# jjjkkyz/NU-NeRF

Measured on AMD Instinct MI355X. Metric: train rays/sec, higher is better.
Workload: dtype f32

## Files before the change

### nu_nerf_amd/csrc/gemm_epi.h

```cpp
#pragma once
#include "gemm.h"
#include <type_traits>

#define TBM 128
#define TBN 128
#define TBK 32
#define NT_LDS 36
#define NT_LDSH 40
#define NT_WPC 3

#define EPI_LDS 68

template <int EPI>
static __device__ inline float nu_epi_apply(float v, float bv, float h, float d, float ca, float& out2) {
    out2 = 0.f;
    if (EPI == NU_EPI_BIAS_NONE) return v + bv;
    if (EPI == NU_EPI_BIAS_RELU) return fmaxf(v + bv, 0.0f);
    if (EPI == NU_EPI_BIAS_SOFTPLUS) return nu_softplus100_fast(v + bv);
    if (EPI == NU_EPI_MUL_DRELU) return h > 0.0f ? v : 0.0f;
    if (EPI == NU_EPI_MUL_DSP) return v * (1.0f - nu_exp_m100(h));
    if (EPI == NU_EPI_Q_SP) {
        const float e = nu_exp_m100(h);
        out2 = v * d * 100.0f * e;
        return v * (1.0f - e);
    }
    if (EPI == NU_EPI_B_SP) return v * (1.0f - nu_exp_m100(h)) + ca;
    if (EPI == NU_EPI_B_RELU) return (h > 0.0f ? v : 0.0f) + ca;
    return v;
}

template <int EPI>
struct NtEpiArgs {
    float* C; float* C2; const float* bias; const float* H; const float* D; const float* Cadd;
    unsigned long long* mask;
    int zero_to, act_cols;
    bool vec_ok;
    bool c16, x16;
    static constexpr bool kMaskW = (EPI == NU_EPI_BIAS_RELU);
    static constexpr bool kMaskR = (EPI == NU_EPI_MUL_DRELU || EPI == NU_EPI_B_RELU);
    static constexpr bool kNeedH = (EPI == NU_EPI_MUL_DRELU || EPI == NU_EPI_MUL_DSP || EPI == NU_EPI_Q_SP ||
                                    EPI == NU_EPI_B_SP || EPI == NU_EPI_B_RELU);
    static constexpr bool kNeedD = (EPI == NU_EPI_Q_SP);
    static constexpr bool kNeedAdd = (EPI == NU_EPI_B_SP || EPI == NU_EPI_B_RELU);
    static constexpr bool kBias = (EPI <= NU_EPI_BIAS_SOFTPLUS);
};

template <int EPI, bool H16 = false>
static __device__ inline NtEpiArgs<EPI> nt_epi_args(const NuGemmNT& g, int z) {
    typedef NtEpiArgs<EPI> E;
    E a;
    a.c16 = H16 && (g.bf16 & NU_GEMM_C16) != 0;
    a.x16 = H16 && (g.bf16 & NU_GEMM_X16) != 0;
    const int ec = a.c16 ? 2 : 4, ex = a.x16 ? 2 : 4;
    auto off = [](const float* p, long long elems, int eb) { return reinterpret_cast<const float*>(reinterpret_cast<const char*>(p) + elems * eb); };
    a.C = const_cast<float*>(off(g.C, (long long)z * g.sC, ec));
    a.C2 = g.C2 ? const_cast<float*>(off(g.C2, (long long)z * g.sC2, ec)) : nullptr;
    a.bias = g.bias ? g.bias + (long long)z * g.sBias : nullptr;
    a.H = g.H ? off(g.H, (long long)z * g.sH, ex) : nullptr;
    a.D = g.D ? off(g.D, (long long)z * g.sD, ex) : nullptr;
    a.Cadd = g.Cadd ? off(g.Cadd, (long long)z * g.sCadd, ex) : nullptr;
    a.zero_to = g.zero_to > g.N ? g.zero_to : g.N;
    a.act_cols = g.act_cols > 0 ? g.act_cols : 0x7fffffff;
    a.mask = (E::kMaskW || E::kMaskR) ? g.mask : nullptr;
    const uintptr_t mc = a.c16 ? 7 : 15, mx = a.x16 ? 7 : 15;
    bool v = (((uintptr_t)a.C & mc) == 0) && ((g.ldc & 3) == 0);
    if (E::kNeedH) v = v && (((uintptr_t)a.H & mx) == 0) && ((g.ldh & 3) == 0);
    if (E::kNeedD) v = v && (((uintptr_t)a.D & mx) == 0) && ((g.ldd & 3) == 0) && (((uintptr_t)a.C2 & mc) == 0) && ((g.ldc2 & 3) == 0);
    if (E::kNeedAdd) v = v && (((uintptr_t)a.Cadd & mx) == 0) && ((g.ldadd & 3) == 0);
    a.vec_ok = v;
    return a;
}

static __device__ __forceinline__ f32x4 nu_bf16x4_to_f32(uint2 r) {
    f32x4 o;
    o[0] = __uint_as_float(r.x << 16); o[1] = __uint_as_float(r.x & 0xffff0000u);
    o[2] = __uint_as_float(r.y << 16); o[3] = __uint_as_float(r.y & 0xffff0000u);
    return o;
}
template <bool H16> static __device__ __forceinline__ f32x4 nt_ld4(const char* p, bool is16) {
    if (H16 && is16) return nu_bf16x4_to_f32(*reinterpret_cast<const uint2*>(p));
    return *reinterpret_cast<const f32x4*>(p);
}
template <bool H16> static __device__ __forceinline__ void nt_st4(char* p, f32x4 v, bool is16) {
// ... 6 lines not shown
}
template <bool H16> static __device__ __forceinline__ void nt_st1(float* base, long long idx, float v, bool is16) {
    if (H16 && is16) reinterpret_cast<__bf16*>(base)[idx] = (__bf16)v;
    else base[idx] = v;
}

template <int EPI>
static __device__ inline unsigned long long* nt_mask_words(const NtEpiArgs<EPI>& ea, const NuGemmNT& g, int mt, int nt, int z, int ntn, int wid) {
    const int ct = g.mask_ct0 + z * ntn + nt;
    return (ea.mask && ct < g.mask_nct) ? ea.mask + ((((long long)mt * g.mask_nct + ct) * 4 + wid) * 64) : nullptr;
}

template <int EPI, int NBH, bool H16 = false, int TMN = 2>
static __device__ __forceinline__ void nt_epilogue(const NuGemmNT& g, const NtEpiArgs<EPI>& ea, f32x16 (&acc)[TMN][2], float* scr,
                                                   int m0, int n0, unsigned long long* mwave, unsigned mlo, unsigned mhi,
                                                   int lane, int wid, int tm0 = 0) {
    typedef NtEpiArgs<EPI> E;
    constexpr bool kMaskW = E::kMaskW, kMaskR = E::kMaskR, kNeedH = E::kNeedH, kNeedD = E::kNeedD, kNeedAdd = E::kNeedAdd, kBias = E::kBias;
    float* const C = ea.C; float* const C2 = ea.C2;
    const float* const bias = ea.bias; const float* const H = ea.H; const float* const D = ea.D; const float* const Cadd = ea.Cadd;
    const int zero_to = ea.zero_to, act_cols = ea.act_cols;
    const bool vec_ok = ea.vec_ok;
    const bool c16 = H16 && ea.c16, x16 = H16 && ea.x16;
    const int ec = c16 ? 2 : 4, ex = x16 ? 2 : 4;
    const int li = lane & 31, lh = lane >> 5;
    const int wr = wid >> 1, wc = wid & 1;
    unsigned wlo = 0, whi = 0;
    const int colq = (lane & 15) * 4;
    const int gcol = n0 + wc * 64 + colq;
    float bv[4] = {0.f, 0.f, 0.f, 0.f};
    if (kBias && bias) {
#pragma unroll
        for (int e = 0; e < 4; ++e) bv[e] = (gcol + e < g.N) ? bias[gcol + e] : 0.f;
    }
    const bool full = vec_ok && (gcol + 3 < g.N) && (gcol + 3 < act_cols || gcol >= act_cols);
    const int wcol0 = n0 + wc * 64, wrow0 = m0 + wr * 64;
    const bool slab_full = vec_ok && (wrow0 + 64 <= g.M) && (wcol0 + 64 <= g.N) && (wcol0 + 64 <= act_cols || wcol0 >= act_cols);
    const bool slab_plain = kNeedH && wcol0 >= act_cols;
    const int uwid = __builtin_amdgcn_readfirstlane(wid);
    const long long urow0 = m0 + (uwid >> 1) * 64, ucol0 = n0 + (uwid & 1) * 64;
    const unsigned lrow = lane >> 4;
    char* const Cu = reinterpret_cast<char*>(C) + (urow0 * g.ldc + ucol0) * ec;
    char* const C2u = kNeedD ? reinterpret_cast<char*>(C2) + (urow0 * g.ldc2 + ucol0) * ec : nullptr;
    const char* const Hu = kNeedH ? reinterpret_cast<const char*>(H) + (urow0 * g.ldh + ucol0) * ex : nullptr;
    const char* const Du = kNeedD ? reinterpret_cast<const char*>(D) + (urow0 * g.ldd + ucol0) * ex : nullptr;
    const char* const Au = kNeedAdd ? reinterpret_cast<const char*>(Cadd) + (urow0 * g.ldadd + ucol0) * ex : nullptr;
    const unsigned oC = (lrow * (unsigned)g.ldc + (unsigned)colq) * (unsigned)ec, oC2 = (lrow * (unsigned)g.ldc2 + (unsigned)colq) * (unsigned)ec;
    const unsigned oH = (lrow * (unsigned)g.ldh + (unsigned)colq) * (unsigned)ex, oD = (lrow * (unsigned)g.ldd + (unsigned)colq) * (unsigned)ex;
    const unsigned oA = (lrow * (unsigned)g.ldadd + (unsigned)colq) * (unsigned)ex;
#pragma unroll
    for (int tt = 0; tt < TMN; ++tt) {
        const int tm = tm0 + tt;
#pragma unroll
        for (int tn = 0; tn < 2; ++tn)
#pragma unroll
            for (int r = 0; r < 16; ++r)
                scr[((r & 3) + 8 * (r >> 2) + 4 * lh) * EPI_LDS + tn * 32 + li] = acc[tt][tn][r];
        if (slab_full) {
            auto fast = [&](auto ub_c, auto pl_c, auto c16_c, auto x16_c) {
                constexpr bool UB = decltype(ub_c)::value, PL = decltype(pl_c)::value;
                constexpr bool c16 = decltype(c16_c)::value, x16 = decltype(x16_c)::value;
                constexpr int ec = c16 ? 2 : 4, ex = x16 ? 2 : 4;
                constexpr int NB = kNeedH ? NBH : 4;
#pragma unroll
                for (int hb = 0; hb < 8 / NB; ++hb) {
                    f32x4 v4[NB], h4[NB], d4[NB], c4v[NB];
#pragma unroll
                    for (int ii = 0; ii < NB; ++ii) {
                        const int i = hb * NB + ii;
                        const long long roff = (long long)(tm * 32 + i * 4);
                        v4[ii] = *reinterpret_cast<const f32x4*>(&scr[(i * 4 + (lane >> 4)) * EPI_LDS + colq]);
                        if (kNeedH && !PL && !UB) h4[ii] = nt_ld4<H16>(Hu + roff * g.ldh * ex + oH, x16);
                        if (kNeedD && !PL) d4[ii] = nt_ld4<H16>(Du + roff * g.ldd * ex + oD, x16);
                        if (kNeedAdd && !PL) c4v[ii] = nt_ld4<H16>(Au + roff * g.ldadd * ex + oA, x16);
                    }
#pragma unroll
                    for (int ii = 0; ii < NB; ++ii) {
                        const int i = hb * NB + ii;
                        const long long roff = (long long)(tm * 32 + i * 4);
                        f32x4 o4, o24;
#pragma unroll
                        for (int e = 0; e < 4; ++e) {
                            float o2 = 0.f;
                            const float v = g.alpha * v4[ii][e];
                            if constexpr (PL) {
                                o4[e] = v;
                            } else if constexpr (kMaskR && UB) {
                                const int src = (tm * 8 + i) * 4 + e;
                                const unsigned long long w = ((unsigned long long)(unsigned)__builtin_amdgcn_readlane(mhi, src) << 32) |
                                                             (unsigned)__builtin_amdgcn_readlane(mlo, src);
                                float sel;
                                asm("s_nop 1\n\tv_cndmask_b32_e64 %0, 0, %1, %2" : "=v"(sel) : "v"(v), "s"(w));
                                o4[e] = kNeedAdd ? sel + c4v[ii][e] : sel;
                            } else {
                                o4[e] = nu_epi_apply<EPI>(v, bv[e], kNeedH ? h4[ii][e] : 0.f, kNeedD ? d4[ii][e] : 0.f,
                                                          kNeedAdd ? c4v[ii][e] : 0.f, o2);
                            }
                            o24[e] = o2;
                        }
                        nt_st4<H16>(Cu + roff * g.ldc * ec + oC, o4, c16);
                        if (kNeedD) nt_st4<H16>(C2u + roff * g.ldc2 * ec + oC2, o24, c16);
                        if constexpr (kMaskW && UB) {
#pragma unroll
                            for (int e = 0; e < 4; ++e) {
                                const unsigned long long bits = __ballot(o4[e] > 0.f);
                                const bool mine = lane == (tm * 8 + i) * 4 + e;
                                wlo = mine ? (unsigned)bits : wlo;
                                whi = mine ? (unsigned)(bits >> 32) : whi;
                            }
                        }
                    }
                }
            };
            auto fast_w = [&](auto ub_c, auto pl_c) {
                constexpr bool kAux = kNeedH || kNeedD || kNeedAdd;
                if constexpr (H16) {
                    if (c16) {
                        if (kAux && x16) fast(ub_c, pl_c, std::true_type{}, std::true_type{});
                        else fast(ub_c, pl_c, std::true_type{}, std::false_type{});
                    } else {
                        if (kAux && x16) fast(ub_c, pl_c, std::false_type{}, std::true_type{});
                        else fast(ub_c, pl_c, std::false_type{}, std::false_type{});
                    }
                } else {
                    fast(ub_c, pl_c, std::false_type{}, std::false_type{});
                }
            };
            if (kNeedH && slab_plain) fast_w(std::false_type{}, std::true_type{});
            else if ((kMaskR || kMaskW) && mwave) fast_w(std::true_type{}, std::false_type{});
            else fast_w(std::false_type{}, std::false_type{});
        } else if (gcol < zero_to) {
#pragma unroll 4
            for (int i = 0; i < 8; ++i) {
                const int rl = i * 4 + (lane >> 4);
                const int row = m0 + wr * 64 + tm * 32 + rl;
                const f32x4 v4 = *reinterpret_cast<const f32x4*>(&scr[rl * EPI_LDS + colq]);
                bool pos[4] = {false, false, false, false};
                if (row < g.M) {
                if (full) {
                    f32x4 h4 = {0.f, 0.f, 0.f, 0.f}, d4 = h4, c4v = h4, o4, o24;
                    const bool plain = gcol >= act_cols;
                    if (kMaskR && mwave) {
                        if (!plain) {
#pragma unroll
                            for (int e = 0; e < 4; ++e) {
                                const int src = (tm * 8 + i) * 4 + e;
                                const unsigned lo = __builtin_amdgcn_readlane(mlo, src), hi = __builtin_amdgcn_readlane(mhi, src);
                                h4[e] = (((lane < 32 ? lo : hi) >> (lane & 31)) & 1u) ? 1.0f : 0.0f;
                            }
                        }
                    } else if (kNeedH && !plain) h4 = nt_ld4<H16>(reinterpret_cast<const char*>(H) + ((long long)row * g.ldh + gcol) * ex, x16);
                    if (kNeedD && !plain) d4 = nt_ld4<H16>(reinterpret_cast<const char*>(D) + ((long long)row * g.ldd + gcol) * ex, x16);
                    if (kNeedAdd && !plain) c4v = nt_ld4<H16>(reinterpret_cast<const char*>(Cadd) + ((long long)row * g.ldadd + gcol) * ex, x16);
#pragma unroll
                    for (int e = 0; e < 4; ++e) {
                        float o2;
                        const float v = g.alpha * v4[e];
                        o4[e] = (kNeedH && plain) ? v : nu_epi_apply<EPI>(v, bv[e], h4[e], d4[e], c4v[e], o2);
                        o24[e] = (kNeedH && plain) ? 0.f : o2;
                    }
                    nt_st4<H16>(reinterpret_cast<char*>(C) + ((long long)row * g.ldc + gcol) * ec, o4, c16);
                    if (kNeedD) nt_st4<H16>(reinterpret_cast<char*>(C2) + ((long long)row * g.ldc2 + gcol) * ec, o24, c16);
                    if (kMaskW) {
#pragma unroll
                        for (int e = 0; e < 4; ++e) pos[e] = o4[e] > 0.f;
                    }
                } else {
#pragma unroll
                    for (int e = 0; e < 4; ++e) {
                        const int col = gcol + e;
                        if (col >= zero_to) continue;
                        float out = 0.f, out2 = 0.f;
                        if (col < g.N) {
                            const float v = g.alpha * v4[e];
                            if (kNeedH && col >= act_cols) {
                                out = v;
                            } else {
                                const float h = kNeedH ? nt_ld1<H16>(H, (long long)row * g.ldh + col, x16) : 0.f;
                                const float d = kNeedD ? nt_ld1<H16>(D, (long long)row * g.ldd + col, x16) : 0.f;
                                const float ca = kNeedAdd ? nt_ld1<H16>(Cadd, (long long)row * g.ldadd + col, x16) : 0.f;
                                out = nu_epi_apply<EPI>(v, bv[e], h, d, ca, out2);
                            }
                        }
                        nt_st1<H16>(C, (long long)row * g.ldc + col, out, c16);
                        if (kNeedD) nt_st1<H16>(C2, (long long)row * g.ldc2 + col, out2, c16);
                    }
                }
                }
                if (kMaskW && mwave) {
#pragma unroll
                    for (int e = 0; e < 4; ++e) {
                        const unsigned long long bits = __ballot(pos[e]);
                        const bool mine = lane == (tm * 8 + i) * 4 + e;
                        wlo = mine ? (unsigned)bits : wlo;
                        whi = mine ? (unsigned)(bits >> 32) : whi;
                    }
                }
            }
        }
    }
    if (kMaskW && mwave && (TMN == 2 || (lane >> 5) == tm0)) mwave[lane] = ((unsigned long long)whi << 32) | wlo;
}

// ... 1 lines not shown
```

### nu_nerf_amd/csrc/gemm_nt.hip

```cpp
#include "gemm_epi.h"

template <int EPI, int PREC>
__global__ __launch_bounds__(256, PREC == 2 ? 2 : NT_WPC) void gemm_nt_kernel(NuGemmNT g) {
    static_assert(PREC == 1 || PREC == 2, "gemm_nt_kernel covers the bf16 modes only");
    constexpr bool SPLIT = PREC == 2;
    constexpr int kPlane = TBM * NT_LDSH;
    __shared__ __attribute__((aligned(16))) float smem[SPLIT ? 1 : 2][SPLIT ? 3 * kPlane : TBM * NT_LDS];
    __bf16* const hA = reinterpret_cast<__bf16*>(&smem[0][0]);
    __bf16* const hB = hA + (SPLIT ? 3 : 1) * kPlane;

    const int tid = threadIdx.x;
    const int lane = tid & 63;
    const int wid = tid >> 6;
    const int wr = wid >> 1, wc = wid & 1;
    const int z = blockIdx.z;
    const int ntn = (g.N + TBN - 1) / TBN;
    const int mtiles = (g.M + TBM - 1) / TBM;
    const int nslots = ((mtiles + 7) / 8) * 8 * ntn;

    const float* __restrict__ A = g.A + (long long)z * g.sA;
    const float* __restrict__ B = g.B + (long long)z * g.sB;
    const int c4 = tid & 7;
    const int r0 = tid >> 3;
    const int nk = g.K / TBK;
// ... 333 lines not shown
template <int EPI, int TMN>
__global__ __launch_bounds__(256, 2) void gemm_nt2b_kernel(NuGemmNTBatch b) {
    __shared__ __attribute__((aligned(16))) float smem[2 * NT2_STAGE];
    nt2_run<EPI, TMN, true>(b.p, b.slot0, b.n, smem);
}

int nu_gemm_nt16_launch(const NuGemmNT& g, int groups, long long nslots, hipStream_t stream);
int nu_gemm_nt6_launch(const NuGemmNT& g, int groups, hipStream_t stream);

static int nt_check(const NuGemmNT& g) {
    if (g.N <= 0 || g.K <= 0 || (g.K % TBK) != 0 || g.lda < g.K || g.ldb < g.K) return NU_ERR_ARG;
    if ((g.lda & 3) || (g.ldb & 3)) return NU_ERR_ARG;
    if (((uintptr_t)g.A & 15) || ((uintptr_t)g.B & 15)) return NU_ERR_ARG;
    const int ntn = nu_cdiv(g.N, TBN);
    const long long nslots = (long long)nu_rup(nu_cdiv(g.M, 64), 8) * ntn;
    if (nslots > 0x7fffffffLL) return NU_ERR_ARG;
    const int groups = g.groups > 0 ? g.groups : 1;
    if (g.mask && (g.epi == NU_EPI_BIAS_RELU || g.epi == NU_EPI_MUL_DRELU || g.epi == NU_EPI_B_RELU)) {
        if ((g.N & 3) || (g.ldc & 3) || ((uintptr_t)g.C & 15) || g.mask_nct <= 0 || g.mask_ct0 < 0) return NU_ERR_ARG;
        if (g.epi == NU_EPI_B_RELU && ((g.ldadd & 3) || ((uintptr_t)g.Cadd & 15))) return NU_ERR_ARG;
        if (g.epi == NU_EPI_BIAS_RELU && ((long long)g.mask_ct0 + (long long)groups * ntn > g.mask_nct || (g.N & 63))) return NU_ERR_ARG;
        if (g.act_cols > 0 && (g.act_cols & 63)) return NU_ERR_ARG;
    }
    const int prec = g.bf16 & 3;
    if (prec == 3) return NU_ERR_ARG;
    if ((g.bf16 & ~3) && !(prec == 1 && (g.bf16 & NU_GEMM_B16)) && !(prec == 2 && (g.bf16 & ~3) == NU_GEMM_PRESPLIT_ALWAYS && g.B6))
        return NU_ERR_ARG;
    return NU_OK;
}

static bool nt_small_tiles(long long t128, long long t64) {
    auto round_eff = [&](long long tiles) { return (double)tiles / (double)(nu_cdivl(tiles, 512) * 512); };
    return t128 < 512 || 0.95 * round_eff(t64) > round_eff(t128);
}

int nu_gemm_nt_launch(const NuGemmNT& g, hipStream_t stream) {
    if (g.M <= 0) return NU_OK;
    const int rc = nt_check(g);
    if (rc != NU_OK) return rc;
    const int ntn = nu_cdiv(g.N, TBN);
    const long long nslots = (long long)nu_rup(nu_cdiv(g.M, TBM), 8) * ntn;
    const int groups = g.groups > 0 ? g.groups : 1;
    const int prec = g.bf16 & 3;
    dim3 block(256);
    if (prec == 1 && (g.bf16 & NU_GEMM_B16)) return nu_gemm_nt16_launch(g, groups, nslots, stream);
    const bool nt6_epi = g.epi != NU_EPI_Q_SP && g.epi != NU_EPI_B_SP && g.epi != NU_EPI_B_RELU;
// ... 116 lines not shown
```

### nu_nerf_amd/csrc/mlp.hip

```cpp
#include "gemm.h"


static __device__ inline int nu_find_desc(const NuPackDesc* __restrict__ d, int nd, int row) {
    int lo = 0, hi = nd - 1;
    while (lo < hi) {
        int mid = (lo + hi + 1) >> 1;
        if (d[mid].row_begin <= row) lo = mid; else hi = mid - 1;
    }
    return lo;
}

__global__ __launch_bounds__(64) void pack_kernel(const NuPackDesc* __restrict__ descs, int nd) {
    const int row = blockIdx.x;
    const int lane = threadIdx.x;
    const NuPackDesc d = descs[nu_find_desc(descs, nd, row)];
    const int n = row - d.row_begin;
    const float* __restrict__ v = d.v + (long long)n * d.K;
    float s = d.scale;
    if (d.g) {
        float ss = 0.f;
        for (int k = lane; k < d.K; k += 64) ss += v[k] * v[k];
        ss = nu_wave_sum(ss);
        s *= d.g[n] / sqrtf(ss);
    }
// ... 205 lines not shown
#pragma unroll
        for (int t = 0; t < KQ; ++t) {
            w[j][t] = *reinterpret_cast<const f32x4*>(Ws + (long long)j * ldw + 4 * ln + 256 * t);
            acc[j][t] = f32x4{0.f, 0.f, 0.f, 0.f};
        }
    }
    constexpr int STEP = 4 * RPW;
    auto row_body = [&](int p, const f32x4* h) {
#pragma clang fp contract(off)
        float g[NO];
#pragma unroll
        for (int j = 0; j < NO; ++j) {
            g[j] = dy[(long long)p * ldy + j];
            bacc[j] += g[j];
        }
#pragma unroll
        for (int t = 0; t < KQ; ++t) {
            f32x4 d = {0.f, 0.f, 0.f, 0.f};
#pragma unroll
            for (int j = 0; j < NO; ++j) {
                d += g[j] * w[j][t];
                acc[j][t] += g[j] * h[t];
            }
            if (relu_mask) {
#pragma unroll
                for (int e = 0; e < 4; ++e) d[e] = h[t][e] > 0.f ? d[e] : 0.f;
            }
            const long long qi = (long long)p * lddh + cb + 4 * ln + 256 * t;
            if (accumulate) d += sk_ld4<H16>(dH, qi);
            sk_st4<H16>(dH, qi, d);
        }
    };
    int p = p0 + wave * RPW + sub;
    for (; p + STEP < p1; p += 2 * STEP) {
        f32x4 ha[KQ], hb[KQ];
#pragma unroll
        for (int t = 0; t < KQ; ++t) {
            ha[t] = sk_ld4<H16>(H, (long long)p * ldh + cb + 4 * ln + 256 * t);
            hb[t] = sk_ld4<H16>(H, (long long)(p + STEP) * ldh + cb + 4 * ln + 256 * t);
        }
        row_body(p, ha);
        row_body(p + STEP, hb);
    }
    for (; p < p1; p += STEP) {
        f32x4 ha[KQ];
#pragma unroll
// ... 35 lines not shown
}

static int skinny_bwd_launch(const float* dy, int ldy, const float* H, int ldh, int P, int K, const float* Ws, int ldw, int NO, float* dH,
                             int lddh, int relu_mask, int accumulate, float* dWs, int lddw, float* db, void* workspace,
                             long long workspace_bytes, NuReduceDesc* descs, int* ndesc, int cap, bool h16, hipStream_t stream);
extern "C" int nu_skinny_bwd_enqueue(const float* dy, int ldy, const float* H, int ldh, int P, int K, const float* Ws,
                                     int ldw, int NO, float* dH, int lddh, int relu_mask, int accumulate, float* dWs,
                                     int lddw, float* db, void* workspace, long long workspace_bytes,
                                     NuReduceDesc* descs, int* ndesc, int cap, hipStream_t stream) {
    return skinny_bwd_launch(dy, ldy, H, ldh, P, K, Ws, ldw, NO, dH, lddh, relu_mask, accumulate, dWs, lddw, db, workspace, workspace_bytes,
                             descs, ndesc, cap, false, stream);
}
extern "C" int nu_skinny_bwd_enqueue_h16(const float* dy, int ldy, const void* H, int ldh, int P, int K, const float* Ws,
                                         int ldw, int NO, void* dH, int lddh, int relu_mask, int accumulate, float* dWs,
                                         int lddw, float* db, void* workspace, long long workspace_bytes,
                                         NuReduceDesc* descs, int* ndesc, int cap, hipStream_t stream) {
    return skinny_bwd_launch(dy, ldy, static_cast<const float*>(H), ldh, P, K, Ws, ldw, NO, static_cast<float*>(dH), lddh, relu_mask,
                             accumulate, dWs, lddw, db, workspace, workspace_bytes, descs, ndesc, cap, true, stream);
}
static int skinny_bwd_launch(const float* dy, int ldy, const float* H, int ldh, int P, int K, const float* Ws, int ldw, int NO, float* dH,
                             int lddh, int relu_mask, int accumulate, float* dWs, int lddw, float* db, void* workspace,
                             long long workspace_bytes, NuReduceDesc* descs, int* ndesc, int cap, bool h16, hipStream_t stream) {
    if (P <= 0) return NU_ERR_ARG;
    if (workspace_bytes < nu_skinny_bwd_workspace_bytes(K, NO)) return NU_ERR_WORKSPACE;
    if (*ndesc + 2 > cap) return NU_ERR_WORKSPACE;
    int blocks = nu_cdiv(P, 64);
    blocks = blocks < NU_SKINNY_BLOCKS ? blocks : NU_SKINNY_BLOCKS;
    float* slab = (float*)workspace;
    float* bslab = slab + (long long)NU_SKINNY_BLOCKS * NO * K;
#define NU_ARGS dy, ldy, H, ldh, P, Ws, ldw, dH, lddh, relu_mask, accumulate, slab, bslab, K
    if ((ldh & 3) || (lddh & 3) || (ldw & 3)) return NU_ERR_ARG;
    if (K == 128) {
        switch (NO) {
            case 1: if (h16) hipLaunchKernelGGL((skinny_bwd_kernel<1, 128, true>), dim3(blocks), dim3(256), 0, stream, NU_ARGS); else hipLaunchKernelGGL((skinny_bwd_kernel<1, 128, false>), dim3(blocks), dim3(256), 0, stream, NU_ARGS); break;
            case 3: if (h16) hipLaunchKernelGGL((skinny_bwd_kernel<3, 128, true>), dim3(blocks), dim3(256), 0, stream, NU_ARGS); else hipLaunchKernelGGL((skinny_bwd_kernel<3, 128, false>), dim3(blocks), dim3(256), 0, stream, NU_ARGS); break;
            default: return NU_ERR_ARG;
        }
    } else if (K == 256) {
        switch (NO) {
            case 1: if (h16) hipLaunchKernelGGL((skinny_bwd_kernel<1, 256, true>), dim3(blocks), dim3(256), 0, stream, NU_ARGS); else hipLaunchKernelGGL((skinny_bwd_kernel<1, 256, false>), dim3(blocks), dim3(256), 0, stream, NU_ARGS); break;
            case 3: if (h16) hipLaunchKernelGGL((skinny_bwd_kernel<3, 256, true>), dim3(blocks), dim3(256), 0, stream, NU_ARGS); else hipLaunchKernelGGL((skinny_bwd_kernel<3, 256, false>), dim3(blocks), dim3(256), 0, stream, NU_ARGS); break;
            case 4: if (h16) return NU_ERR_ARG; hipLaunchKernelGGL((skinny_bwd_kernel<4, 256, false>), dim3(blocks), dim3(256), 0, stream, NU_ARGS); break;
            default: return NU_ERR_ARG;
        }
    } else if (K == 1024) {
        switch (NO) {
// ... 149 lines not shown
```

### nu_nerf_amd/csrc/mlp_ops.hip

```cpp
#include "gemm.h"

#define CHK(x) do { const int rc_ = (x); if (rc_ != NU_OK) return rc_; } while (0)

extern "C" int nu_skinny_fwd(const float*, int, int, int, const float*, int, const float*, int, float*, int, hipStream_t);
extern "C" int nu_skinny_fwd_h16(const void*, int, int, int, const float*, int, const float*, int, float*, int, hipStream_t);
extern "C" int nu_skinny_bwd_enqueue_h16(const float*, int, const void*, int, int, int, const float*, int, int, void*, int, int, int,
                                         float*, int, float*, void*, long long, NuReduceDesc*, int*, int, hipStream_t);
extern "C" long long nu_skinny_bwd_workspace_bytes(int, int);
extern "C" int nu_skinny_bwd_enqueue(const float*, int, const float*, int, int, int, const float*, int, int, float*, int, int, int,
                                     float*, int, float*, void*, long long, NuReduceDesc*, int*, int, hipStream_t);
extern "C" long long nu_colsum_workspace_bytes(int);
extern "C" int nu_colsum_enqueue(const float*, int, int, int, float*, int, void*, long long, NuReduceDesc*, int*, int, hipStream_t);
extern "C" int nu_rowscale_dsp(const float*, int, int, int, const float*, float*, int, hipStream_t);
extern "C" long long nu_wgrad_workspace_bytes(int, int, int, int);
extern "C" int nu_wgrad_enqueue(const NuGemmTN*, float*, int, long long, float*, long long, void*, long long, NuReduceDesc*, int*, int,
                                hipStream_t);

static inline int rup_i(int a, int b) { return (a + b - 1) / b * b; }

extern "C" int nu_op_ctx_size(void) { return (int)sizeof(NuOpCtx); }

static inline int ctx_take(NuOpCtx* c, long long nbytes, int ndesc_needed, hipStream_t stream, float** out, long long* out_bytes) {
    return nu_ctx_take(c, nbytes, ndesc_needed, stream, out, out_bytes);
}
// ... 17 lines not shown
    long long sA = 0, sB = 0, sC = 0, sBias = 0, sH = 0; unsigned long long* mask = nullptr; int mask_nct = 0;
    const float* B16 = nullptr;
    int st = 0;
    int ktrue = 0;
};
static int nt_fill(const NuOpCtx* c, const NtArgs& a, NuGemmNT& g) {
    const bool h16 = c->h16 != 0;
    if (h16 && (c->prec != 1 || a.B16 == nullptr)) return NU_ERR_ARG;
    g = NuGemmNT{};
    g.A = a.A; g.lda = a.lda; g.B = h16 ? a.B16 : a.B; g.ldb = a.ldb; g.M = a.M; g.N = a.N; g.K = a.K; g.C = a.C; g.ldc = a.ldc; g.C2 = a.C2;
    g.ldc2 = a.ldc2; g.bias = a.bias; g.H = a.H; g.ldh = a.ldh; g.D = a.D; g.ldd = a.ldd; g.Cadd = a.Cadd; g.ldadd = a.ldadd;
    g.zero_to = a.zero_to; g.act_cols = a.act_cols; g.alpha = 1.0f; g.groups = a.groups; g.sA = a.sA; g.sB = a.sB; g.sC = a.sC;
    g.sBias = a.sBias; g.sH = a.sH; g.epi = a.epi; g.bf16 = h16 ? (1 | NU_GEMM_B16 | a.st) : c->prec; g.mask = a.mask;
    g.mask_nct = a.mask ? a.mask_nct : 0;
    if (c->prec == 2 && !h16) g.B6 = a.B16;
    return NU_OK;
}
static void nt_cost(const NuOpCtx* c, const NtArgs& a, double* flops, double* bytes) {
    const bool h16 = c->h16 != 0;
    const double eA = h16 && (a.st & A16) ? 2 : 4, eB = h16 ? 2 : 4, eC = h16 && (a.st & C16) ? 2 : 4, eX = h16 && (a.st & X16) ? 2 : 4;
    const bool mask_r = a.mask && (a.epi == NU_EPI_MUL_DRELU || a.epi == NU_EPI_B_RELU);
    const double K = a.ktrue ? a.ktrue : a.K, M = a.M, N = a.N;
    *bytes += a.groups * (M * K * eA + N * K * eB + M * N * (eC * (1 + (a.C2 ? 1 : 0)) +
                          eX * ((a.H && !mask_r ? 1 : 0) + (a.D ? 1 : 0) + (a.Cadd ? 1 : 0))));
    *flops += 2.0 * M * N * K * a.groups;
}
static int nt(NuOpCtx* c, const NtArgs& a, hipStream_t stream) {
    if (a.M <= 0) return NU_OK;
    NuGemmNT g;
    CHK(nt_fill(c, a, g));
    ev_begin(c, stream);
    const int rc = nu_gemm_nt_launch(g, stream);
    if (c->ev) {
        double flops = 0, bytes = 0;
        nt_cost(c, a, &flops, &bytes);
        ev_end(c, stream, 0.0, flops, bytes);
    }
    return rc;
}
static int nt_batch(NuOpCtx* c, const NtArgs* a, int n, hipStream_t stream) {
    NuGemmNT g[16];
    if (n > 16) return NU_ERR_ARG;
    int m = 0;
    double flops = 0, bytes = 0;
    for (int i = 0; i < n; ++i) {
        if (a[i].M <= 0) continue;
        CHK(nt_fill(c, a[i], g[m++]));
// ... 218 lines not shown
    }
    CHK(skinny_fwd(c, b->H[8], 256, P, 256, net->alpha.Wp, 256, net->alpha.bias, 1, b->sig, 1, stream, true));
    NtArgs gf = {b->H[8], 256, net->feat.Wp, 256, P, 256, 256, b->V, 288, NU_EPI_BIAS_NONE};
    gf.bias = net->feat.bias; gf.B16 = w16(c, net->feat.Wp16, 0); gf.st = A16;
    CHK(nt(c, gf, stream));
    NtArgs gv = {b->V, 288, net->view.Wp, 288, P, 128, 288, b->HV, 128, NU_EPI_BIAS_RELU};
    gv.bias = net->view.bias; gv.B16 = w16(c, net->view.Wp16, 0);
    CHK(nt(c, gv, stream));
    return nu_skinny_fwd(b->HV, 128, P, 128, net->rgb.Wp, 128, net->rgb.bias, 3, b->rgb, 4, stream);
}

extern "C" int nu_nerfpp_mlp_bwd(NuOpCtx* c, const NuNerfNet* net, const float* pt, int pt_ld, NuNerfBufs* b, const float* dsig,
                                 const float* drgb, hipStream_t stream) {
    const int P = b->P;
    if (P <= 0) return NU_OK;
    const bool want_in = b->dx != nullptr;
    const int ldf = want_in ? 288 : 256;
    CHK(skinny_bwd(c, drgb, 4, b->HV, 128, P, 128, net->rgb.Wp, 128, 3, b->dHV, 128, 1, net->rgb.dWp, 128, c->flat + net->rgb.db_off, stream));
    CHK(wgrad(c, b->dHV, 128, b->V, 288, P, 128, 288, net->view.dWp, 288, c->flat + net->view.db_off, stream));
    NtArgs gF = {b->dHV, 128, net->view.WpT, net->view.ldT, P, ldf, 128, b->dF, ldf, NU_EPI_PLAIN};
    gF.B16 = w16(c, net->view.WpT16, 0);
    CHK(nt(c, gF, stream));
    CHK(wgrad(c, b->dF, ldf, b->H[8], 256, P, 256, 256, net->feat.dWp, 256, c->flat + net->feat.db_off, stream, NU_TN_B0_16));
    CHK(skinny_bwd(c, dsig, 1, b->H[8], 256, P, 256, net->alpha.Wp, 256, 1, b->dH8a, 256, 1, net->alpha.dWp, 256, c->flat + net->alpha.db_off, stream,
                   true));
    NtArgs g8 = {b->dF, ldf, net->feat.WpT, net->feat.ldT, P, 256, 256, b->dA[8], 256, NU_EPI_B_RELU};
    g8.H = b->H[8]; g8.ldh = 256; g8.Cadd = b->dH8a; g8.ldadd = 256; g8.mask = b->mask[8]; g8.mask_nct = 2;
    g8.B16 = w16(c, net->feat.WpT16, 0); g8.st = C16 | X16;
    CHK(nt(c, g8, stream));
    const float* dA = b->dA[8];
    int lda = 256;
    int dA_i = 8;
    const float* dskip = nullptr;
    for (int i = 7; i >= 0; --i) {
        const NuLin& L = net->pts[i];
        const int ldu = i == 0 ? 96 : (i == 5 ? 352 : 256);
        CHK(wgrad(c, dA, lda, b->H[i], ldu, P, 256, L.Kp, L.dWp, L.ldd, c->flat + L.db_off, stream,
                  (nerfdA16(dA_i) ? NU_TN_A0_16 : 0) | (nerfH16(i) ? NU_TN_B0_16 : 0)));
        if (i > 0) {
            const int st = (nerfdA16(dA_i) ? A16 : 0) | (nerfdA16(i) ? C16 : 0) | (nerfH16(i) ? X16 : 0);
            if (i == 5 && want_in) {
                NtArgs g = {dA, lda, L.WpT, L.ldT, P, 340, 256, b->dA[i], 352, NU_EPI_MUL_DRELU};
                g.H = b->H[i]; g.ldh = ldu; g.act_cols = 256; g.zero_to = 352; g.mask = b->mask[i]; g.mask_nct = 2;
                g.B16 = w16(c, L.WpT16, 0); g.st = st;
                CHK(nt(c, g, stream));
                dskip = b->dA[i];
                dA = b->dA[i]; lda = 352;
            } else {
                NtArgs g = {dA, lda, L.WpT, L.ldT, P, 256, 256, b->dA[i], 256, NU_EPI_MUL_DRELU};
                g.H = b->H[i]; g.ldh = ldu; g.mask = b->mask[i]; g.mask_nct = 2;
// ... 89 lines not shown
```

### nu_nerf_amd/engine.py

```python
import ctypes
import os
import math

import numpy as np
import torch

from . import _lib as L

from ._lib import (GemmNT, GemmTN, ReduceDesc, PackDesc, Lin, WgradItem, OpCtx, SdfNet, SdfBufs, NerfNet, NerfBufs, ShadeNet, BakeNet,
                   ShadeBufs, EPI_BIAS_NONE, EPI_BIAS_RELU, EPI_BIAS_SOFTPLUS, EPI_MUL_DRELU, EPI_MUL_DSP, EPI_Q_SP, EPI_B_SP,
                   EPI_PLAIN, EPI_B_RELU, NU_WGRAD_QUEUE_MAX)

c_int, c_p = ctypes.c_int, ctypes.c_void_p


def rup(a, b):
    return (a + b - 1) // b * b


def addr(t, off=0):
    if t is None:
        return 0
    return t.data_ptr() + t.element_size() * off

# ... 410 lines not shown
            for l in layers:
                if l.row_begin != row0 + rows:
                    raise ValueError("unpack_grads(layers=...): the layers are not consecutive in the descriptor table")
                rows += l.N
            rng = self._unpack_ranges[key] = (layers, row0, rows)
        self.lib.nu_unpack_grads_range(self._desc_dev.data_ptr(), len(self.layers), rng[1], rng[2], flat.data_ptr(), self.stream())

    def nt(self, A, lda, B, ldb, M, N, K, C, ldc, epi, *, C2=0, ldc2=0, bias=0, H=0, ldh=0, D=0, ldd=0, Cadd=0,
           ldadd=0, zero_to=0, act_cols=0, alpha=1.0, groups=1, sA=0, sB=0, sC=0, sC2=0, sBias=0, sH=0, sD=0, sCadd=0,
           ktrue=None, ntrue=None, mask=None, B6=0):
        if M <= 0:
            return
        g = GemmNT(A, lda, B, ldb, M, N, K, C, ldc, C2, ldc2, bias, H, ldh, D, ldd, Cadd, ldadd, zero_to, act_cols,
                   alpha, groups, sA, sB, sC, sC2, sBias, sH, sD, sCadd, epi, self.bf16,
                   mask.data_ptr() if mask is not None else 0, mask._nu_nct if mask is not None else 0, 0, B6)
        kt = self._ktime if self.ktime_on else None
        if kt is not None:
            e0, e1 = self._event_pair()
            e0.record()
        self.lib.nu_gemm_nt_ex(ctypes.byref(g), self.stream())
        if kt is not None:
            e1.record()
            reads_h = bool(H) and not (mask is not None and epi in (EPI_MUL_DRELU, EPI_B_RELU))
            nmat = 1 + (1 if C2 else 0) + (1 if reads_h else 0) + (1 if D else 0) + (1 if Cadd else 0)
            abytes = 4.0 * groups * (M * (ktrue or K) + M * (ntrue or N) * nmat + N * (ktrue or K))
            kt['nt'].append((e0, e1, 2.0 * M * (ntrue or N) * (ktrue or K) * groups, abytes))

    def nt_desc(self, A, lda, B, ldb, M, N, K, C, ldc, epi, *, C2=0, ldc2=0, bias=0, H=0, ldh=0, D=0, ldd=0, Cadd=0, ldadd=0, zero_to=0,
                act_cols=0, alpha=1.0, groups=1, sA=0, sB=0, sC=0, sC2=0, sBias=0, sH=0, sD=0, sCadd=0, mask=None):
        return GemmNT(A, lda, B, ldb, M, N, K, C, ldc, C2, ldc2, bias, H, ldh, D, ldd, Cadd, ldadd, zero_to, act_cols,
                      alpha, groups, sA, sB, sC, sC2, sBias, sH, sD, sCadd, epi, self.bf16,
                      mask.data_ptr() if mask is not None else 0, mask._nu_nct if mask is not None else 0, 0, 0)

    def nt_batch(self, descs):
        descs = [g for g in descs if g.M > 0]
        if not descs:
            return
        arr = (GemmNT * len(descs))(*descs)
        kt = self._ktime if self.ktime_on else None
        if kt is not None:
            e0, e1 = self._event_pair()
            e0.record()
        self.lib.nu_gemm_nt_batch(arr, len(descs), self.stream())
        if kt is not None:
            e1.record()
            fl = by = 0.0
            for g in descs:
                nmat = 1 + (1 if g.C2 else 0) + (1 if (g.H and not (g.mask and g.epi in (EPI_MUL_DRELU, EPI_B_RELU))) else 0) + (1 if g.D else 0) + (1 if g.Cadd else 0)
                fl += 2.0 * g.M * g.N * g.K * g.groups
                by += 4.0 * g.groups * (g.M * g.K + g.M * g.N * nmat + g.N * g.K)
            kt['nt'].append((e0, e1, fl, by))

    def begin_kernel_timing(self, reserve=0, py_reserve=None):
        self._ktime = {'nt': [], 'tn': []}
        n = max(int(reserve), 4) // 4 * 4
        if py_reserve is None:
            py_reserve = n if self.py_seq else n // 4
        py_reserve = min(max(int(py_reserve), 0) // 2 * 2, n)
        pool = [torch.cuda.Event(enable_timing=True) for _ in range(n)]
        for ev in pool:
            ev.record()
        torch.cuda.synchronize(self.dev)
        n_c = 0 if self.py_seq else n - py_reserve
        self._ev_c = pool[:n_c]
        self._ev_pool = pool[n_c:]
        self._ev_py_exhausted = False
        self._ev_handles = (c_p * max(n_c, 1))(*[ev.cuda_event for ev in self._ev_c])
        self._ev_meta = (ctypes.c_double * (3 * max(n_c // 2, 1)))()
        self._ctx.nev, self._ctx.ev_cap, self._ctx.ev_meta = 0, n_c, ctypes.addressof(self._ev_meta)
        self.ktime_on = True

# ... 564 lines not shown
        if alpha_rm is not None:
            lib.nu_nerf_act_fwd(addr(sig), 1, addr(rgb), 4, addr(pt), addr(idx), P, addr(alpha_rm), addr(color_rm), S)
        b.update(V=V, HV=HV, sig=sig, rgb=rgb)
        return b

    def nerf_backward(self, b, pt, idx, dalpha_rm, dcolor_rm, flat, dsig=None, drgb=None, dx=None, ddir=None):
        lib, S, P = self.lib, self.stream(), b['P']
        e = self.empty
        H = b['H']
        want_in = dx is not None
        if dsig is None:
            dsig, drgb = e(P), e(P, 4)
            lib.nu_nerf_act_bwd(addr(b['sig']), 1, addr(b['rgb']), 4, addr(pt), addr(idx), P,
                                addr(dalpha_rm), addr(dcolor_rm), addr(dsig), 1, addr(drgb), 4, S)
        if self._use_c():
            cb = b.get('cb')
            if cb is None:
                cb = NerfBufs(P=P, V=addr(b['V']), HV=addr(b['HV']), sig=addr(b['sig']), rgb=addr(b['rgb']))
                for i in range(9):
                    cb.H[i] = addr(H[i])
                    if i > 0:
                        cb.mask[i] = addr(getattr(H[i], '_nu_mask', None))
            ldf = 288 if want_in else 256
            keep = [e(P, 128), e(P, ldf), self.empty_h(P, 256)]
            cb.dHV, cb.dF, cb.dH8a = (addr(t) for t in keep)
            for i in range(1, 9):
                t = e(P, 352 if want_in else 256) if i == 5 else self.empty_h(P, 256)
                keep.append(t)
                cb.dA[i] = addr(t)
            if want_in:
                t = e(P, 96)
                keep.append(t)
                cb.dE4, cb.dx, cb.ddir = addr(t), addr(dx), addr(ddir)
            else:
                cb.dE4 = cb.dx = cb.ddir = 0
            self._ensure_arena()
            self._ctx.flat = addr(flat)
            lib.nu_nerfpp_mlp_bwd(ctypes.byref(self._ctx), ctypes.byref(self._nerf_net), addr(pt),
                                  pt.shape[1], ctypes.byref(cb), addr(dsig), addr(drgb), S)
            return
        with self.wgrad_batch() as wb:
            dHV = wb.keep(e(P, 128))
            self.skinny_bwd(addr(drgb), 4, addr(b['HV']), 128, P, 128, addr(*self.nerf_rgb.Wp), 128, 3, addr(dHV), 128, 1, 0,
                            addr(*self.nerf_rgb.dWp), 128, addr(flat, self.nerf_rgb.db_off))
            self.wgrad(addr(dHV), 128, addr(b['V']), 288, P, 128, 288, addr(*self.nerf_view.dWp), 288,
                       addr(flat, self.nerf_view.db_off))
            ldf = 288 if want_in else 256
            dF = wb.keep(e(P, ldf))
            self.nt(addr(dHV), 128, addr(*self.nerf_view.WpT), self.nerf_view.ldT, P, ldf, 128, addr(dF), ldf, EPI_PLAIN)
            self.wgrad(addr(dF), ldf, addr(H[8]), 256, P, 256, 256, addr(*self.nerf_feat.dWp), 256,
                       addr(flat, self.nerf_feat.db_off))
            dH8a = wb.keep(e(P, 256))
            self.skinny_bwd(addr(dsig), 1, addr(H[8]), 256, P, 256, addr(*self.nerf_alpha.Wp), 256, 1, addr(dH8a), 256, 1, 0,
                            addr(*self.nerf_alpha.dWp), 256, addr(flat, self.nerf_alpha.db_off))
            dA = wb.keep(e(P, 256))
            self.nt(addr(dF), ldf, addr(*self.nerf_feat.WpT), self.nerf_feat.ldT, P, 256, 256, addr(dA), 256, EPI_B_RELU,
                    H=addr(H[8]), ldh=256, Cadd=addr(dH8a), ldadd=256, mask=getattr(H[8], '_nu_mask', None))
            dskip, lda = None, 256
            for i in range(7, -1, -1):
                lay = self.nerf[i]
                ldu = 96 if i == 0 else (352 if i == 5 else 256)
                self.wgrad(addr(dA), lda, addr(H[i]), ldu, P, 256, lay.Kp, addr(*lay.dWp), lay.ldd, addr(flat, lay.db_off))
                if i > 0:
                    if i == 5 and want_in:
                        nxt = wb.keep(e(P, 352))
                        self.nt(addr(dA), lda, addr(*lay.WpT), lay.ldT, P, 340, 256, addr(nxt), 352, EPI_MUL_DRELU,
                                H=addr(H[i]), ldh=ldu, act_cols=256, zero_to=352, mask=getattr(H[i], '_nu_mask', None))
                        dskip = nxt
                        dA, lda = nxt, 352
                    else:
                        nxt = wb.keep(e(P, 256))
                        self.nt(addr(dA), lda, addr(*lay.WpT), lay.ldT, P, 256, 256, addr(nxt), 256, EPI_MUL_DRELU,
                                H=addr(H[i]), ldh=ldu, mask=getattr(H[i], '_nu_mask', None))
                        dA, lda = nxt, 256
                elif want_in:
                    dE4 = wb.keep(e(P, 96))
                    self.nt(addr(dA), lda, addr(*lay.WpT), lay.ldT, P, 84, 256, addr(dE4), 96, EPI_PLAIN, zero_to=96)
                    lib.nu_nerf_embed_bwd(addr(pt), pt.shape[1], addr(H[0]), addr(b['V']), addr(dE4), 96,
                                          addr(dskip, 256), 352, addr(dF, 256), ldf, P, addr(dx), addr(ddir), S)

# ... 212 lines not shown
```

Measured before the change: 98330.

## Fuse alpha-head rank-1 gradient into B_RELU GEMM epilogue instead of materializing dH8a

The alpha head's backward contribution to dH8 is the outer product dsig[row] * Wp_alpha[col]. Previously the skinny backward wrote it to a full P×256 buffer that the feature GEMM epilogue then read back. Now the skinny kernel skips writing dH when the pointer is null, and the B_RELU epilogue recomputes the product from dsig and the weight vector, passed through the D and bias slots. This removes one full-size write and read of an activation gradient, at the cost of more epilogue code paths and reuse of the D/bias fields with new meaning.

```diff
diff --git a/nu_nerf_amd/csrc/gemm_epi.h b/nu_nerf_amd/csrc/gemm_epi.h
--- a/nu_nerf_amd/csrc/gemm_epi.h
+++ b/nu_nerf_amd/csrc/gemm_epi.h
@@ -28,6 +28,15 @@
     if (EPI == NU_EPI_B_RELU) return (h > 0.0f ? v : 0.0f) + ca;
     return v;
 }
+static __device__ __forceinline__ float nu_rank1_mul(float d, float w) {
+#pragma clang fp contract(off)
+    return d * w;
+}
+static __device__ __forceinline__ float nu_rank1_add(float v, float d, float w) {
+#pragma clang fp contract(off)
+    const float p = d * w;
+    return v + p;
+}
 
 template <int EPI>
 struct NtEpiArgs {
@@ -36,6 +45,7 @@
     int zero_to, act_cols;
     bool vec_ok;
     bool c16, x16;
+    bool rank1;
     static constexpr bool kMaskW = (EPI == NU_EPI_BIAS_RELU);
     static constexpr bool kMaskR = (EPI == NU_EPI_MUL_DRELU || EPI == NU_EPI_B_RELU);
     static constexpr bool kNeedH = (EPI == NU_EPI_MUL_DRELU || EPI == NU_EPI_MUL_DSP || EPI == NU_EPI_Q_SP ||
@@ -59,6 +69,7 @@
     a.H = g.H ? off(g.H, (long long)z * g.sH, ex) : nullptr;
     a.D = g.D ? off(g.D, (long long)z * g.sD, ex) : nullptr;
     a.Cadd = g.Cadd ? off(g.Cadd, (long long)z * g.sCadd, ex) : nullptr;
+    a.rank1 = EPI == NU_EPI_B_RELU && g.Cadd == nullptr;
     a.zero_to = g.zero_to > g.N ? g.zero_to : g.N;
     a.act_cols = g.act_cols > 0 ? g.act_cols : 0x7fffffff;
     a.mask = (E::kMaskW || E::kMaskR) ? g.mask : nullptr;
@@ -111,6 +122,7 @@
     const int zero_to = ea.zero_to, act_cols = ea.act_cols;
     const bool vec_ok = ea.vec_ok;
     const bool c16 = H16 && ea.c16, x16 = H16 && ea.x16;
+    const bool rank1 = !H16 && EPI == NU_EPI_B_RELU && ea.rank1;
     const int ec = c16 ? 2 : 4, ex = x16 ? 2 : 4;
     const int li = lane & 31, lh = lane >> 5;
     const int wr = wid >> 1, wc = wid & 1;
@@ -137,6 +149,8 @@
     const unsigned oC = (lrow * (unsigned)g.ldc + (unsigned)colq) * (unsigned)ec, oC2 = (lrow * (unsigned)g.ldc2 + (unsigned)colq) * (unsigned)ec;
     const unsigned oH = (lrow * (unsigned)g.ldh + (unsigned)colq) * (unsigned)ex, oD = (lrow * (unsigned)g.ldd + (unsigned)colq) * (unsigned)ex;
     const unsigned oA = (lrow * (unsigned)g.ldadd + (unsigned)colq) * (unsigned)ex;
+    const char* const Dr = rank1 ? reinterpret_cast<const char*>(D + urow0) : nullptr;
+    const char* const Wr = rank1 ? reinterpret_cast<const char*>(bias + ucol0) : nullptr;
 #pragma unroll
     for (int tt = 0; tt < TMN; ++tt) {
         const int tm = tm0 + tt;
@@ -145,15 +159,27 @@
 #pragma unroll
             for (int r = 0; r < 16; ++r)
                 scr[((r & 3) + 8 * (r >> 2) + 4 * lh) * EPI_LDS + tn * 32 + li] = acc[tt][tn][r];
-        if (slab_full) {
-            auto fast = [&](auto ub_c, auto pl_c, auto c16_c, auto x16_c) {
+        if (slab_full && !(rank1 && !mwave)) {
+            auto fast = [&](auto ub_c, auto pl_c, auto c16_c, auto x16_c, auto r1_c) {
                 constexpr bool UB = decltype(ub_c)::value, PL = decltype(pl_c)::value;
+                constexpr bool R1 = !H16 && EPI == NU_EPI_B_RELU && decltype(r1_c)::value && UB && !PL;
                 constexpr bool c16 = decltype(c16_c)::value, x16 = decltype(x16_c)::value;
                 constexpr int ec = c16 ? 2 : 4, ex = x16 ? 2 : 4;
                 constexpr int NB = kNeedH ? NBH : 4;
+                float w1[4];
+                unsigned oW = (unsigned)colq * 4u, oR = lrow * 4u;
+                const char* Db = nullptr;
+                if constexpr (R1) {
+                    asm volatile("" : "+v"(oW), "+v"(oR));
+                    const f32x4 w4 = *reinterpret_cast<const f32x4*>(Wr + oW);
+#pragma unroll
+                    for (int e = 0; e < 4; ++e) w1[e] = w4[e];
+                    Db = Dr + __builtin_amdgcn_readfirstlane(tm) * 128;
+                }
 #pragma unroll
                 for (int hb = 0; hb < 8 / NB; ++hb) {
                     f32x4 v4[NB], h4[NB], d4[NB], c4v[NB];
+                    float d1[NB];
 #pragma unroll
                     for (int ii = 0; ii < NB; ++ii) {
                         const int i = hb * NB + ii;
@@ -161,7 +187,8 @@
                         v4[ii] = *reinterpret_cast<const f32x4*>(&scr[(i * 4 + (lane >> 4)) * EPI_LDS + colq]);
                         if (kNeedH && !PL && !UB) h4[ii] = nt_ld4<H16>(Hu + roff * g.ldh * ex + oH, x16);
                         if (kNeedD && !PL) d4[ii] = nt_ld4<H16>(Du + roff * g.ldd * ex + oD, x16);
-                        if (kNeedAdd && !PL) c4v[ii] = nt_ld4<H16>(Au + roff * g.ldadd * ex + oA, x16);
+                        if (kNeedAdd && !PL && !R1) c4v[ii] = nt_ld4<H16>(Au + roff * g.ldadd * ex + oA, x16);
+                        if (R1) d1[ii] = *reinterpret_cast<const float*>(Db + i * 16 + oR);
                     }
 #pragma unroll
                     for (int ii = 0; ii < NB; ++ii) {
@@ -178,9 +205,10 @@
                                 const int src = (tm * 8 + i) * 4 + e;
                                 const unsigned long long w = ((unsigned long long)(unsigned)__builtin_amdgcn_readlane(mhi, src) << 32) |
                                                              (unsigned)__builtin_amdgcn_readlane(mlo, src);
+                                const float vs = R1 ? nu_rank1_add(v, d1[ii], w1[e]) : v;
                                 float sel;
-                                asm("s_nop 1\n\tv_cndmask_b32_e64 %0, 0, %1, %2" : "=v"(sel) : "v"(v), "s"(w));
-                                o4[e] = kNeedAdd ? sel + c4v[ii][e] : sel;
+                                asm("s_nop 1\n\tv_cndmask_b32_e64 %0, 0, %1, %2" : "=v"(sel) : "v"(vs), "s"(w));
+                                o4[e] = (kNeedAdd && !R1) ? sel + c4v[ii][e] : sel;
                             } else {
                                 o4[e] = nu_epi_apply<EPI>(v, bv[e], kNeedH ? h4[ii][e] : 0.f, kNeedD ? d4[ii][e] : 0.f,
                                                           kNeedAdd ? c4v[ii][e] : 0.f, o2);
@@ -201,19 +229,26 @@
                     }
                 }
             };
-            auto fast_w = [&](auto ub_c, auto pl_c) {
+            auto fast_x = [&](auto ub_c, auto pl_c, auto r1_c) {
                 constexpr bool kAux = kNeedH || kNeedD || kNeedAdd;
                 if constexpr (H16) {
                     if (c16) {
-                        if (kAux && x16) fast(ub_c, pl_c, std::true_type{}, std::true_type{});
-                        else fast(ub_c, pl_c, std::true_type{}, std::false_type{});
+                        if (kAux && x16) fast(ub_c, pl_c, std::true_type{}, std::true_type{}, r1_c);
+                        else fast(ub_c, pl_c, std::true_type{}, std::false_type{}, r1_c);
                     } else {
-                        if (kAux && x16) fast(ub_c, pl_c, std::false_type{}, std::true_type{});
-                        else fast(ub_c, pl_c, std::false_type{}, std::false_type{});
+                        if (kAux && x16) fast(ub_c, pl_c, std::false_type{}, std::true_type{}, r1_c);
+                        else fast(ub_c, pl_c, std::false_type{}, std::false_type{}, r1_c);
                     }
                 } else {
-                    fast(ub_c, pl_c, std::false_type{}, std::false_type{});
-                }
+                    fast(ub_c, pl_c, std::false_type{}, std::false_type{}, r1_c);
+                }
+            };
+            auto fast_w = [&](auto ub_c, auto pl_c) {
+                constexpr bool kR1 = !H16 && EPI == NU_EPI_B_RELU && decltype(ub_c)::value && !decltype(pl_c)::value;
+                if constexpr (kR1) {
+                    if (rank1) { fast_x(ub_c, pl_c, std::true_type{}); return; }
+                }
+                fast_x(ub_c, pl_c, std::false_type{});
             };
             if (kNeedH && slab_plain) fast_w(std::false_type{}, std::true_type{});
             else if ((kMaskR || kMaskW) && mwave) fast_w(std::true_type{}, std::false_type{});
@@ -240,7 +275,13 @@
                         }
                     } else if (kNeedH && !plain) h4 = nt_ld4<H16>(reinterpret_cast<const char*>(H) + ((long long)row * g.ldh + gcol) * ex, x16);
                     if (kNeedD && !plain) d4 = nt_ld4<H16>(reinterpret_cast<const char*>(D) + ((long long)row * g.ldd + gcol) * ex, x16);
-                    if (kNeedAdd && !plain) c4v = nt_ld4<H16>(reinterpret_cast<const char*>(Cadd) + ((long long)row * g.ldadd + gcol) * ex, x16);
+                    if (rank1) {
+                        if (!plain) {
+                            const float dr = D[row];
+#pragma unroll
+                            for (int e = 0; e < 4; ++e) c4v[e] = h4[e] > 0.0f ? nu_rank1_mul(dr, bias[gcol + e]) : 0.0f;
+                        }
+                    } else if (kNeedAdd && !plain) c4v = nt_ld4<H16>(reinterpret_cast<const char*>(Cadd) + ((long long)row * g.ldadd + gcol) * ex, x16);
 #pragma unroll
                     for (int e = 0; e < 4; ++e) {
                         float o2;
@@ -267,7 +308,8 @@
                             } else {
                                 const float h = kNeedH ? nt_ld1<H16>(H, (long long)row * g.ldh + col, x16) : 0.f;
                                 const float d = kNeedD ? nt_ld1<H16>(D, (long long)row * g.ldd + col, x16) : 0.f;
-                                const float ca = kNeedAdd ? nt_ld1<H16>(Cadd, (long long)row * g.ldadd + col, x16) : 0.f;
+                                const float ca = rank1 ? (h > 0.0f ? nu_rank1_mul(D[row], bias[gcol + e]) : 0.0f)
+                                                 : kNeedAdd ? nt_ld1<H16>(Cadd, (long long)row * g.ldadd + col, x16) : 0.f;
                                 out = nu_epi_apply<EPI>(v, bv[e], h, d, ca, out2);
                             }
                         }
diff --git a/nu_nerf_amd/csrc/gemm_nt.hip b/nu_nerf_amd/csrc/gemm_nt.hip
--- a/nu_nerf_amd/csrc/gemm_nt.hip
+++ b/nu_nerf_amd/csrc/gemm_nt.hip
@@ -379,6 +379,9 @@
         if (g.epi == NU_EPI_BIAS_RELU && ((long long)g.mask_ct0 + (long long)groups * ntn > g.mask_nct || (g.N & 63))) return NU_ERR_ARG;
         if (g.act_cols > 0 && (g.act_cols & 63)) return NU_ERR_ARG;
     }
+    if (g.epi == NU_EPI_B_RELU && g.Cadd == nullptr &&
+        (g.D == nullptr || g.bias == nullptr || g.ldd != 0 || ((uintptr_t)g.bias & 15) || (groups > 1 && (g.sBias & 3)) || (g.bf16 & NU_GEMM_B16)))
+        return NU_ERR_ARG;
     const int prec = g.bf16 & 3;
     if (prec == 3) return NU_ERR_ARG;
     if ((g.bf16 & ~3) && !(prec == 1 && (g.bf16 & NU_GEMM_B16)) && !(prec == 2 && (g.bf16 & ~3) == NU_GEMM_PRESPLIT_ALWAYS && g.B6))
diff --git a/nu_nerf_amd/csrc/mlp.hip b/nu_nerf_amd/csrc/mlp.hip
--- a/nu_nerf_amd/csrc/mlp.hip
+++ b/nu_nerf_amd/csrc/mlp.hip
@@ -251,6 +251,7 @@
                 d += g[j] * w[j][t];
                 acc[j][t] += g[j] * h[t];
             }
+            if (dH == nullptr) continue;
             if (relu_mask) {
 #pragma unroll
                 for (int e = 0; e < 4; ++e) d[e] = h[t][e] > 0.f ? d[e] : 0.f;
@@ -332,6 +333,7 @@
                              int lddh, int relu_mask, int accumulate, float* dWs, int lddw, float* db, void* workspace,
                              long long workspace_bytes, NuReduceDesc* descs, int* ndesc, int cap, bool h16, hipStream_t stream) {
     if (P <= 0) return NU_ERR_ARG;
+    if (dH == nullptr && accumulate) return NU_ERR_ARG;
     if (workspace_bytes < nu_skinny_bwd_workspace_bytes(K, NO)) return NU_ERR_WORKSPACE;
     if (*ndesc + 2 > cap) return NU_ERR_WORKSPACE;
     int blocks = nu_cdiv(P, 64);
diff --git a/nu_nerf_amd/csrc/mlp_ops.hip b/nu_nerf_amd/csrc/mlp_ops.hip
--- a/nu_nerf_amd/csrc/mlp_ops.hip
+++ b/nu_nerf_amd/csrc/mlp_ops.hip
@@ -63,7 +63,7 @@
     const bool mask_r = a.mask && (a.epi == NU_EPI_MUL_DRELU || a.epi == NU_EPI_B_RELU);
     const double K = a.ktrue ? a.ktrue : a.K, M = a.M, N = a.N;
     *bytes += a.groups * (M * K * eA + N * K * eB + M * N * (eC * (1 + (a.C2 ? 1 : 0)) +
-                          eX * ((a.H && !mask_r ? 1 : 0) + (a.D ? 1 : 0) + (a.Cadd ? 1 : 0))));
+                          eX * ((a.H && !mask_r ? 1 : 0) + (a.D && a.epi != NU_EPI_B_RELU ? 1 : 0) + (a.Cadd ? 1 : 0))));
     *flops += 2.0 * M * N * K * a.groups;
 }
 static int nt(NuOpCtx* c, const NtArgs& a, hipStream_t stream) {
@@ -328,10 +328,13 @@
     gF.B16 = w16(c, net->view.WpT16, 0);
     CHK(nt(c, gF, stream));
     CHK(wgrad(c, b->dF, ldf, b->H[8], 256, P, 256, 256, net->feat.dWp, 256, c->flat + net->feat.db_off, stream, NU_TN_B0_16));
-    CHK(skinny_bwd(c, dsig, 1, b->H[8], 256, P, 256, net->alpha.Wp, 256, 1, b->dH8a, 256, 1, net->alpha.dWp, 256, c->flat + net->alpha.db_off, stream,
+    float* const dH8a = c->h16 ? b->dH8a : nullptr;
+    CHK(skinny_bwd(c, dsig, 1, b->H[8], 256, P, 256, net->alpha.Wp, 256, 1, dH8a, 256, 1, net->alpha.dWp, 256, c->flat + net->alpha.db_off, stream,
                    true));
     NtArgs g8 = {b->dF, ldf, net->feat.WpT, net->feat.ldT, P, 256, 256, b->dA[8], 256, NU_EPI_B_RELU};
-    g8.H = b->H[8]; g8.ldh = 256; g8.Cadd = b->dH8a; g8.ldadd = 256; g8.mask = b->mask[8]; g8.mask_nct = 2;
+    g8.H = b->H[8]; g8.ldh = 256; g8.mask = b->mask[8]; g8.mask_nct = 2;
+    if (dH8a) { g8.Cadd = dH8a; g8.ldadd = 256; }
+    else { g8.D = dsig; g8.ldd = 0; g8.bias = net->alpha.Wp; }
     g8.B16 = w16(c, net->feat.WpT16, 0); g8.st = C16 | X16;
     CHK(nt(c, g8, stream));
     const float* dA = b->dA[8];
diff --git a/nu_nerf_amd/engine.py b/nu_nerf_amd/engine.py
--- a/nu_nerf_amd/engine.py
+++ b/nu_nerf_amd/engine.py
@@ -456,7 +456,7 @@
         if kt is not None:
             e1.record()
             reads_h = bool(H) and not (mask is not None and epi in (EPI_MUL_DRELU, EPI_B_RELU))
-            nmat = 1 + (1 if C2 else 0) + (1 if reads_h else 0) + (1 if D else 0) + (1 if Cadd else 0)
+            nmat = 1 + (1 if C2 else 0) + (1 if reads_h else 0) + (1 if (D and epi != EPI_B_RELU) else 0) + (1 if Cadd else 0)
             abytes = 4.0 * groups * (M * (ktrue or K) + M * (ntrue or N) * nmat + N * (ktrue or K))
             kt['nt'].append((e0, e1, 2.0 * M * (ntrue or N) * (ktrue or K) * groups, abytes))
 
@@ -480,7 +480,7 @@
             e1.record()
             fl = by = 0.0
             for g in descs:
-                nmat = 1 + (1 if g.C2 else 0) + (1 if (g.H and not (g.mask and g.epi in (EPI_MUL_DRELU, EPI_B_RELU))) else 0) + (1 if g.D else 0) + (1 if g.Cadd else 0)
+                nmat = 1 + (1 if g.C2 else 0) + (1 if (g.H and not (g.mask and g.epi in (EPI_MUL_DRELU, EPI_B_RELU))) else 0) + (1 if (g.D and g.epi != EPI_B_RELU) else 0) + (1 if g.Cadd else 0)
                 fl += 2.0 * g.M * g.N * g.K * g.groups
                 by += 4.0 * g.groups * (g.M * g.K + g.M * g.N * nmat + g.N * g.K)
             kt['nt'].append((e0, e1, fl, by))
@@ -1091,8 +1091,12 @@
                     if i > 0:
                         cb.mask[i] = addr(getattr(H[i], '_nu_mask', None))
             ldf = 288 if want_in else 256
-            keep = [e(P, 128), e(P, ldf), self.empty_h(P, 256)]
-            cb.dHV, cb.dF, cb.dH8a = (addr(t) for t in keep)
+            keep = [e(P, 128), e(P, ldf)]
+            cb.dHV, cb.dF = (addr(t) for t in keep)
+            cb.dH8a = 0
+            if self.h16:
+                keep.append(self.empty_h(P, 256))
+                cb.dH8a = addr(keep[-1])
             for i in range(1, 9):
                 t = e(P, 352 if want_in else 256) if i == 5 else self.empty_h(P, 256)
                 keep.append(t)
@@ -1119,12 +1123,12 @@
             self.nt(addr(dHV), 128, addr(*self.nerf_view.WpT), self.nerf_view.ldT, P, ldf, 128, addr(dF), ldf, EPI_PLAIN)
             self.wgrad(addr(dF), ldf, addr(H[8]), 256, P, 256, 256, addr(*self.nerf_feat.dWp), 256,
                        addr(flat, self.nerf_feat.db_off))
-            dH8a = wb.keep(e(P, 256))
-            self.skinny_bwd(addr(dsig), 1, addr(H[8]), 256, P, 256, addr(*self.nerf_alpha.Wp), 256, 1, addr(dH8a), 256, 1, 0,
+            self.skinny_bwd(addr(dsig), 1, addr(H[8]), 256, P, 256, addr(*self.nerf_alpha.Wp), 256, 1, 0, 256, 1, 0,
                             addr(*self.nerf_alpha.dWp), 256, addr(flat, self.nerf_alpha.db_off))
             dA = wb.keep(e(P, 256))
             self.nt(addr(dF), ldf, addr(*self.nerf_feat.WpT), self.nerf_feat.ldT, P, 256, 256, addr(dA), 256, EPI_B_RELU,
-                    H=addr(H[8]), ldh=256, Cadd=addr(dH8a), ldadd=256, mask=getattr(H[8], '_nu_mask', None))
+                    H=addr(H[8]), ldh=256, D=addr(dsig), ldd=0, bias=addr(*self.nerf_alpha.Wp),
+                    mask=getattr(H[8], '_nu_mask', None))
             dskip, lda = None, 256
             for i in range(7, -1, -1):
                 lay = self.nerf[i]
```

Result: no change. 98550 (median of 4 runs) (+0.2%).
